# wangchou/whisper.coreml

Measured on AMD Instinct MI355X. Metric: xRT (audio-s/s) large-v3 beam=5 @1/2/4/8 GPU; p50 per-token decode ms, higher is better.
Workload: dtype fp16; 1 GPU; large-v3 beam=5 transcribe() of one 600 s file, 30 s clip grid, condition_on_previous_text=False, temperature=0; model=large-v3, global_batch=20, seq_len=448

## Files before the change

__graft_entry__.py:

```python
import os
import subprocess
import sys

REPO = os.path.dirname(os.path.abspath(__file__))
PKG = os.path.join(REPO, "whisper.coreml_amd")


def _paths():
    for p in (PKG, REPO):
        if p not in sys.path:
            sys.path.insert(0, p)


def build() -> None:
    env = dict(os.environ)
    env.setdefault("PYTORCH_ROCM_ARCH", "gfx950")
    jobs = str(min(8, os.cpu_count() or 4))
    subprocess.run(["make", "-C", PKG, "-j" + jobs, "ARCH=gfx950"], check=True, env=env)
    _paths()
    import whisper
    from whisper import backend_hip
    backend_hip.load_library()


def smoke() -> None:
    _paths()
    import numpy as np
    import torch

    import whisper
    from whisper import synthetic as S
    from whisper.decoding import DecodingOptions, decode
    from oracle import ref_whisper as R

    dims = S.MODEL_DIMS["micro"]
    sd = S.synthetic_state_dict(dims, 0)
    model = whisper.Whisper(whisper.ModelDimensions(**dims), "micro", device=0, dtype="fp32",
                            max_windows=1, max_group=1)
    model.load_state_dict(sd)
    audio = S.synthetic_audio(30.0, seed=3)

    mel = whisper.log_mel_spectrogram(audio, dims["n_mels"], padding=whisper.audio.N_SAMPLES)
    mel = whisper.pad_or_trim(mel[:, :3000], 3000)
    ref_mel = R.pad_or_trim(R.log_mel_spectrogram(audio, dims["n_mels"], padding=R.N_SAMPLES)[:, :3000]).numpy()
    err = float(np.abs(mel - ref_mel).max())
    assert err < 2e-3, f"log-mel max abs err {err}"

    om = R.OracleWhisper(dims, sd)
    xa_ref = om.encode(torch.from_numpy(mel)).numpy()
    model.ctx.mel_write(mel)
    model.ctx.encode([0], [3000])
    xa = model.ctx.audio_features(0)
    err = float(np.abs(xa - xa_ref.reshape(xa.shape)).max())
    assert err < 2e-3, f"audio features max abs err {err}"

    st = R.SpecialTokens.for_model(dims)
    om.set_audio(torch.from_numpy(xa_ref))
    ref_logits, _, _ = om.decoder_forward(torch.tensor([list(st.sot_sequence)]), 0, None)
    logits, _ = model.ctx.prefill_logits(0, list(st.sot_sequence))
    err = float(np.abs(logits[-1] - ref_logits[0, -1].numpy()).max())
    assert err < 2e-3, f"first-pass logits max abs err {err}"

    opts = DecodingOptions(language="en", sample_len=24, without_timestamps=True)
    res = decode(model, mel, opts)
    ref = R.decode(om, torch.from_numpy(mel), R.Options(sample_len=24, without_timestamps=True), st,
                   xa=torch.from_numpy(xa_ref))
    assert list(res.tokens) == list(ref.tokens), (res.tokens, ref.tokens)
    model.close()
    print(f"smoke ok: {len(res.tokens)} tokens match the oracle")


if __name__ == "__main__":
    build()
    if len(sys.argv) > 1 and sys.argv[1] == "smoke":
        smoke()
```

whisper.coreml_amd/csrc/wh_gemm.h:

```cpp
#pragma once
#include "wh_common.h"

namespace wh {

enum Epi {
  EPI_STORE = 0,
  EPI_STORE_GELU = 1,
  EPI_RESID = 2,
  EPI_GELU_POS = 3,
  EPI_HEADSPLIT = 4,
  EPI_QKV_DEC = 5,
  EPI_F32_COLS = 6,
  EPI_PARTIAL = 7,
  EPI_QKV_ENC = 8,
};

struct GemmArgs {
  const void* X = nullptr;
  const void* W = nullptr;
  const float* bias = nullptr;
  int M = 0, N = 0, K = 0;
  int ldx = 0;
  int x_group_rows = 1 << 30;
  int64_t x_group_stride = 0;
  void* out = nullptr;
  float* out_f32 = nullptr;
  int ldo = 0;
  int64_t out_group_stride = 0;
  int out_row_off = 0;
  const float* pos = nullptr;
  int hs_state = 0, hs_heads = 0, hs_T = 0, hs_nslots = 0, hs_slot0 = 0;
  const int* row_win = nullptr;
  const int* row_slot = nullptr;
  const int* row_pos = nullptr;
  void* kc = nullptr;
  void* vc = nullptr;
  int kv_beams = 0, kv_ctx = 0;
  const int* x_rows = nullptr;
  int ksplit = 1;
  int mt_block = 0;
  int row_groups = 1;
  const float* xf32 = nullptr;
  const float* ln_g = nullptr;
  const float* ln_b = nullptr;
  float ln_eps = 1e-5f;
  float* p1_slab = nullptr;
  int* p1_cnt = nullptr;
  int p1_slabs = 0;
  int p1_defer = 0;
  const float* res_slab = nullptr;
  const float* res_bias = nullptr;
  float* x_out = nullptr;
  int slab_half = 0;
};

template <typename T, int EPI>
WH_DEV void epilogue_store(const GemmArgs& a, int m, int gi, int ri, int n, float4_t v) {
  if constexpr (EPI == EPI_STORE || EPI == EPI_STORE_GELU) {
    if constexpr (EPI == EPI_STORE_GELU) {
#pragma unroll
      for (int j = 0; j < 4; ++j) v[j] = gelu_f(v[j]);
    }
    T* o = reinterpret_cast<T*>(a.out) + (int64_t)gi * a.out_group_stride + (int64_t)(ri + a.out_row_off) * a.ldo + n;
    store4(o, v[0], v[1], v[2], v[3]);
  } else if constexpr (EPI == EPI_RESID) {
    float* o = a.out_f32 + (int64_t)m * a.ldo + n;
    float4_t c = load4f(o);
    c += v;
    store4(o, c[0], c[1], c[2], c[3]);
  } else if constexpr (EPI == EPI_GELU_POS) {
    const float4_t p = load4f(a.pos + (int64_t)ri * a.N + n);
    float* o = a.out_f32 + (int64_t)m * a.ldo + n;
    store4(o, gelu_f(v[0]) + p[0], gelu_f(v[1]) + p[1], gelu_f(v[2]) + p[2], gelu_f(v[3]) + p[3]);
  } else if constexpr (EPI == EPI_HEADSPLIT) {
    const int l2 = n / a.hs_state, c = n - l2 * a.hs_state, h = c >> 6, d = c & 63;
    const int64_t blk = (((int64_t)l2 * a.hs_nslots + a.hs_slot0 + gi) * a.hs_heads + h) * a.hs_T * 64;
    T* o = reinterpret_cast<T*>(a.out) + blk;
    if ((l2 & 1) == 0) {
      store4(o + (int64_t)ri * 64 + d, v[0], v[1], v[2], v[3]);
    } else {
#pragma unroll
      for (int j = 0; j < 4; ++j) o[xv_index(d + j, ri)] = from_f32<T>(v[j]);
    }
  } else if constexpr (EPI == EPI_QKV_ENC) {
    if (n < 2 * a.hs_state) {
      T* o = reinterpret_cast<T*>(a.out) + (int64_t)gi * a.out_group_stride + (int64_t)ri * a.ldo + n;
      store4(o, v[0], v[1], v[2], v[3]);
    } else {
      const int c = n - 2 * a.hs_state, h = c >> 6, d = c & 63;
      const int q = ri & 31;
      const int pt = (ri & ~31) + 8 * ((q & 15) >> 2) + 4 * (q >> 4) + (q & 3);
      T* o = reinterpret_cast<T*>(a.vc) + (((int64_t)gi * a.hs_heads + h) * 64 + d) * a.hs_T + pt;
#pragma unroll
      for (int j = 0; j < 4; ++j) o[(int64_t)j * a.hs_T] = from_f32<T>(v[j]);
    }
  } else if constexpr (EPI == EPI_QKV_DEC) {
    const int ns = a.hs_state;
    if (n < ns) {
      store4(reinterpret_cast<T*>(a.out) + (int64_t)m * a.ldo + n, v[0], v[1], v[2], v[3]);
    } else {
      const int which = n >= 2 * ns;
      const int c = n - ns * (1 + which), h = c >> 6, d = c & 63;
      const int w = a.row_win[m], sl = a.row_slot[m], p = a.row_pos[m];
      const int64_t idx = ((((int64_t)w * a.kv_beams + sl) * a.hs_heads + h) * a.kv_ctx + p) * 64 + d;
      T* base = reinterpret_cast<T*>(which ? a.vc : a.kc);
      store4(base + idx, v[0], v[1], v[2], v[3]);
    }
  }
}

template <typename T, int EPI, int MI, int NI, int MG, typename RowF, typename ColF>
WH_DEV void tile_epilogue(const GemmArgs& a, const float4_t (&acc)[MI][NI], RowF mrow, ColF ncol) {
  static_assert(MI % MG == 0, "row-tile groups");
  constexpr bool LD = EPI == EPI_RESID || EPI == EPI_GELU_POS;
  float4_t bv[NI];
#pragma unroll
  for (int ni = 0; ni < NI; ++ni) bv[ni] = a.bias ? load4f(a.bias + ncol(ni)) : (float4_t){0.f, 0.f, 0.f, 0.f};
#pragma unroll
  for (int g0 = 0; g0 < MI; g0 += MG) {
    float4_t xv[LD ? MG : 1][LD ? NI : 1];
    if constexpr (LD) {
#pragma unroll
      for (int j = 0; j < MG; ++j) {
        const int m = mrow(g0 + j);
        const int gi = m / a.x_group_rows, ri = m - gi * a.x_group_rows;
#pragma unroll
        for (int ni = 0; ni < NI; ++ni) {
          xv[j][ni] = (float4_t){0.f, 0.f, 0.f, 0.f};
          if (m < a.M) {
            if constexpr (EPI == EPI_RESID) xv[j][ni] = load4f(a.out_f32 + (int64_t)m * a.ldo + ncol(ni));
            else xv[j][ni] = load4f(a.pos + (int64_t)ri * a.N + ncol(ni));
          }
        }
      }
    }
#pragma unroll
    for (int j = 0; j < MG; ++j) {
      const int m = mrow(g0 + j);
      if (m >= a.M) continue;
      const int gi = m / a.x_group_rows, ri = m - gi * a.x_group_rows;
#pragma unroll
      for (int ni = 0; ni < NI; ++ni) {
        const int n = ncol(ni);
        float4_t v = acc[g0 + j][ni];
        if (a.bias) v += bv[ni];
        if constexpr (EPI == EPI_RESID) {
          float4_t c = xv[j][ni];
          c += v;
          store4(a.out_f32 + (int64_t)m * a.ldo + n, c[0], c[1], c[2], c[3]);
        } else if constexpr (EPI == EPI_GELU_POS) {
          const float4_t p = xv[j][ni];
          store4(a.out_f32 + (int64_t)m * a.ldo + n, gelu_f(v[0]) + p[0], gelu_f(v[1]) + p[1], gelu_f(v[2]) + p[2],
                 gelu_f(v[3]) + p[3]);
        } else {
          epilogue_store<T, EPI>(a, m, gi, ri, n, v);
        }
      }
    }
  }
}

template <typename T>
int launch_gemm(const GemmArgs& a, int epi, hipStream_t st);
template <typename T>
int launch_gemm_tiles(const GemmArgs& a, int epi, int tile_sel, hipStream_t st);

template <typename T>
int launch_proj_partial(const GemmArgs& a, int max_z, hipStream_t st, int* z_out, hipEvent_t ev0 = nullptr,
                        hipEvent_t ev1 = nullptr);

bool proj1_supported(int R, int n);
template <typename T>
int launch_proj1(const GemmArgs& a, int epi, bool ln, hipStream_t st, hipEvent_t ev0 = nullptr,
                 hipEvent_t ev1 = nullptr);

int gemv_ksplit(int M, int N, int K, int max_z = 16, int mt_block = 0);

}
```

whisper.coreml_amd/csrc/wh_gemm.hip:

```cpp
#include "wh_gemm.h"

#include <algorithm>
#include <type_traits>
#include <cstdlib>

namespace wh {

constexpr int TBM = 128, TBN = 128, TKB = 128;
constexpr int TROW = TKB + 16;

template <typename T, int EPI, int TBN_ = TBN, int KZ = 1>
__global__ __launch_bounds__(256, 2) void k_gemm_tile(GemmArgs a) {
  static_assert(KZ == 1 || KZ == 2, "two K halves at most (their sum commutes)");
  constexpr int BK = TKB / (int)sizeof(T);
  constexpr int KS = BK / 32;
  constexpr int WCH = TBN_ / 32;
  constexpr int NI = TBN_ / 32;
  __shared__ __attribute__((aligned(16))) char smem[2][(TBM + TBN_) * TROW];

  const int ntn = a.N / TBN_;
  const int ntm = (a.M + TBM - 1) / TBM;
  const int rid = xcd_remap(blockIdx.x, ntm * ntn * KZ);
  const int bid = rid / KZ, kz = rid - bid * KZ;
  const int tm = bid / ntn, tn = bid % ntn;
// ... 59 lines not shown
      for (int mi = 0; mi < 4; ++mi)
#pragma unroll
        for (int ni = 0; ni < NI; ++ni) mfma_step(acc[mi][ni], wf[ni], xf[mi]);
    }
  };

  const int nk = a.K / BK / KZ;
  gload(0, ra);
  gload(min(1, nk - 1), rb);
  sstore(0, ra);
  lds_barrier();
  for (int kt = 0; kt < nk; kt += 2) {
    gload(min(kt + 2, nk - 1), ra);
    compute(0);
    if (kt + 1 < nk) sstore(1, rb);
    lds_barrier();
    if (kt + 1 >= nk) break;
    gload(min(kt + 3, nk - 1), rb);
    compute(1);
    if (kt + 2 < nk) sstore(0, ra);
    lds_barrier();
  }

  if constexpr (KZ > 1) {
    constexpr int NE = 4 * NI;
    const int slot = bid * 4 + wave, nslot = ntm * ntn * 4;
    const auto rs = wt_rsrc(a.p1_slab);
    auto off = [&](int z, int e) { return (((z * nslot + slot) * NE + e) * 64 + lane) * 16; };
#pragma unroll
    for (int mi = 0; mi < 4; ++mi)
#pragma unroll
      for (int ni = 0; ni < NI; ++ni) wt_store4(rs, off(kz, mi * NI + ni), acc[mi][ni]);
    asm volatile("s_waitcnt vmcnt(0)" ::: "memory");
    int ticket = 0;
    if (lane == 0) ticket = __hip_atomic_fetch_add(a.p1_cnt + slot, 1, __ATOMIC_RELAXED, __HIP_MEMORY_SCOPE_AGENT);
    ticket = __shfl(ticket, 0, 64);
    if (ticket != KZ - 1) return;
    __builtin_amdgcn_fence(__ATOMIC_ACQUIRE, "wavefront");
    if (lane == 0) __hip_atomic_store(a.p1_cnt + slot, 0, __ATOMIC_RELAXED, __HIP_MEMORY_SCOPE_AGENT);
    float4_t pv[4][NI];
#pragma unroll
    for (int mi = 0; mi < 4; ++mi)
#pragma unroll
      for (int ni = 0; ni < NI; ++ni)
        pv[mi][ni] = __builtin_bit_cast(float4_t, __builtin_amdgcn_raw_buffer_load_b128(rs, off(1 - kz, mi * NI + ni), 0, 16));
#pragma unroll
    for (int mi = 0; mi < 4; ++mi)
#pragma unroll
      for (int ni = 0; ni < NI; ++ni) acc[mi][ni] += pv[mi][ni];
  }

  tile_epilogue<T, EPI, 4, NI, 2>(
      a, acc, [&](int mi) { return m0 + wr * 64 + mi * 16 + r; },
      [&](int ni) { return n0 + wc * (TBN_ / 2) + ni * 16 + 4 * g; });
}

namespace g256 {
constexpr int BM = 256, BN = 256, BK = 64;
constexpr int STAGE = 16384;
constexpr int BUF = 4 * STAGE;
enum { SA0 = 0, SA1 = 1, SB0 = 2, SB1 = 3 };
}

WH_DEV void raw_barrier() {
  asm volatile("" ::: "memory");
  __builtin_amdgcn_sched_barrier(0);
  __builtin_amdgcn_s_barrier();
  __builtin_amdgcn_sched_barrier(0);
  asm volatile("" ::: "memory");
}

WH_DEV void glds16(const char* src, char* lds) {
  __builtin_amdgcn_global_load_lds((__attribute__((address_space(1))) void*)(src),
                                   (__attribute__((address_space(3))) void*)(lds), 16, 0, 0);
}

template <int EPI, int MF = 16>
__global__ __launch_bounds__(512, 1) void k_gemm_256(GemmArgs a) {
  using namespace g256;
  __shared__ __attribute__((aligned(1024))) char smem[2 * BUF];

  const int ntn = a.N / BN;
  const int ntm = (a.M + BM - 1) / BM;
  const int bid = xcd_remap(blockIdx.x, ntm * ntn);
  const int tm = bid / ntn, tn = bid % ntn;
  const int m0 = tm * BM, n0 = tn * BN;
  const int tid = threadIdx.x, lane = tid & 63, wave = tid >> 6;
  const int wr = wave >> 2, wc = wave & 3;
  const int r = lane & 15, g = lane >> 4;

  const int srow = lane >> 2;
  const int schunk = (lane & 3) ^ ((lane >> 5) << 1);
  const half_t* X = reinterpret_cast<const half_t*>(a.X);
  const half_t* W = reinterpret_cast<const half_t*>(a.W);
  const char* src[4];
#pragma unroll
  for (int h = 0; h < 2; ++h) {
    int m = m0 + (wave >> 2) * 128 + h * 64 + (wave & 3) * 16 + srow;
    if (m >= a.M) m = a.M - 1;
    const int gi = m / a.x_group_rows, ri = m - gi * a.x_group_rows;
    src[SA0 + h] = reinterpret_cast<const char*>(X + (int64_t)gi * a.x_group_stride + (int64_t)ri * a.ldx) + schunk * 16;
    const int n = n0 + (wave >> 1) * 64 + h * 32 + (wave & 1) * 16 + srow;
    src[SB0 + h] = reinterpret_cast<const char*>(W + (int64_t)n * a.K) + schunk * 16;
  }
  auto stage = [&](int buf, int st, int kt) {
    const char* s = src[st] + kt * (BK * 2);
    char* d = smem + buf * BUF + st * STAGE + wave * 2048;
    glds16(s, d);
    glds16(s + 64, d + 1024);
  };

  const int roff = r * 64 + ((g ^ ((r >> 3) << 1)) << 4);
  Frag<half_t> af[4][2], bf[2][2];
  auto read_a = [&](int buf, int h) {
    const char* base = smem + buf * BUF + (SA0 + h) * STAGE + wr * 8192 + roff;
#pragma unroll
    for (int mi = 0; mi < 4; ++mi)
#pragma unroll
      for (int ks = 0; ks < 2; ++ks) af[mi][ks].v = *reinterpret_cast<const half8_t*>(base + (mi * 2 + ks) * 1024);
  };
  auto read_b = [&](int buf, int h) {
    const char* base = smem + buf * BUF + (SB0 + h) * STAGE + wc * 4096 + roff;
#pragma unroll
    for (int j = 0; j < 2; ++j)
#pragma unroll
      for (int ks = 0; ks < 2; ++ks) bf[j][ks].v = *reinterpret_cast<const half8_t*>(base + (j * 2 + ks) * 1024);
  };

  const int rr = lane & 15, hb = (lane >> 4) & 1, kh = lane >> 5;
  const int coff0 = rr * 64 + (((0 + kh) ^ ((rr >> 3) << 1)) << 4);
  const int coff1 = rr * 64 + (((2 + kh) ^ ((rr >> 3) << 1)) << 4);
  Frag<half_t> af32[MF == 32 ? 2 : 1][4], bf32[4];
  auto read_a32 = [&](int buf, int h) {
    const char* base = smem + buf * BUF + (SA0 + h) * STAGE + wr * 8192;
#pragma unroll
    for (int t = 0; t < 2; ++t)
#pragma unroll
      for (int st = 0; st < 4; ++st)
        af32[t][st].v = *reinterpret_cast<const half8_t*>(base + ((t * 2 + hb) * 2 + (st >> 1)) * 1024 +
                                                             ((st & 1) ? coff1 : coff0));
  };
  auto read_b32 = [&](int buf, int h) {
    const char* base = smem + buf * BUF + (SB0 + h) * STAGE + wc * 4096;
#pragma unroll
    for (int st = 0; st < 4; ++st)
      bf32[st].v = *reinterpret_cast<const half8_t*>(base + (hb * 2 + (st >> 1)) * 1024 + ((st & 1) ? coff1 : coff0));
  };
  typedef float f32x16_t __attribute__((ext_vector_type(16)));
  f32x16_t acc32[MF == 32 ? 4 : 1][2];
  float4_t acc[MF == 32 ? 1 : 8][4];
  if constexpr (MF == 32) {
#pragma unroll
    for (int i = 0; i < 4; ++i)
#pragma unroll
      for (int j = 0; j < 2; ++j) acc32[i][j] = (f32x16_t){};
  } else {
#pragma unroll
    for (int i = 0; i < 8; ++i)
#pragma unroll
      for (int j = 0; j < 4; ++j) acc[i][j] = (float4_t){0.f, 0.f, 0.f, 0.f};
  }
  auto rd_a = [&](int buf, int h) {
    if constexpr (MF == 32) read_a32(buf, h);
    else read_a(buf, h);
  };
  auto rd_b = [&](int buf, int h) {
    if constexpr (MF == 32) read_b32(buf, h);
    else read_b(buf, h);
  };

  auto mfma_quadrant = [&](int mh, int nh) {
    asm volatile("s_waitcnt lgkmcnt(0)" ::: "memory");
    __builtin_amdgcn_s_setprio(1);
    if constexpr (MF == 32) {
#pragma unroll
      for (int t = 0; t < 2; ++t)
#pragma unroll
        for (int st = 0; st < 4; ++st)
          acc32[mh * 2 + t][nh] =
              __builtin_amdgcn_mfma_f32_32x32x16_f16(bf32[st].v, af32[t][st].v, acc32[mh * 2 + t][nh], 0, 0, 0);
    } else {
#pragma unroll
      for (int mi = 0; mi < 4; ++mi)
#pragma unroll
        for (int j = 0; j < 2; ++j)
#pragma unroll
          for (int ks = 0; ks < 2; ++ks) mfma_step(acc[mh * 4 + mi][nh * 2 + j], bf[j][ks], af[mi][ks]);
    }
    __builtin_amdgcn_s_setprio(0);
  };

  const int nk = a.K / BK;
  auto ktile = [&](auto bufc, int t) {
    constexpr int buf = decltype(bufc)::value;
    const bool s1 = t + 1 < nk, s2 = t + 2 < nk;
    rd_b(buf, 0);
    rd_a(buf, 0);
    if (s1) stage(buf ^ 1, SA1, t + 1);
    raw_barrier();
    mfma_quadrant(0, 0);
    raw_barrier();
    rd_b(buf, 1);
    if (s1) stage(buf ^ 1, SB0, t + 1);
    raw_barrier();
    mfma_quadrant(0, 1);
    raw_barrier();
    rd_a(buf, 1);
    if (s2) stage(buf, SA0, t + 2);
    raw_barrier();
    mfma_quadrant(1, 1);
    raw_barrier();
    rd_b(buf, 0);
    if (s2) {
      stage(buf, SB1, t + 2);
      asm volatile("s_waitcnt vmcnt(4)" ::: "memory");
    } else {
      asm volatile("s_waitcnt vmcnt(0)" ::: "memory");
    }
    raw_barrier();
    mfma_quadrant(1, 0);
    raw_barrier();
  };

  stage(0, SA0, 0);
  stage(0, SB1, 0);
  stage(0, SA1, 0);
  stage(0, SB0, 0);
  stage(1, SA0, 1);
  stage(1, SB1, 1);
  asm volatile("s_waitcnt vmcnt(4)" ::: "memory");
  raw_barrier();
  if (wr == 1) raw_barrier();
  for (int t = 0; t < nk; t += 2) {
    ktile(std::integral_constant<int, 0>(), t);
    ktile(std::integral_constant<int, 1>(), t + 1);
  }
  if (wr == 0) raw_barrier();

  if constexpr (MF == 32) {
    float4_t a4[4][8];
#pragma unroll
    for (int mt = 0; mt < 4; ++mt)
#pragma unroll
      for (int j = 0; j < 8; ++j) {
        const int nt = j >> 2, q = j & 3;
        a4[mt][j] = (float4_t){acc32[mt][nt][4 * q], acc32[mt][nt][4 * q + 1], acc32[mt][nt][4 * q + 2],
                               acc32[mt][nt][4 * q + 3]};
      }
    tile_epilogue<half_t, EPI, 4, 8, 2>(
        a, a4, [&](int mt) { return m0 + wr * 128 + mt * 32 + (lane & 31); },
        [&](int j) { return n0 + wc * 64 + (j >> 2) * 32 + 8 * (j & 3) + 4 * kh; });
  } else {
    tile_epilogue<half_t, EPI, 8, 4, 4>(
        a, acc, [&](int mi) { return m0 + wr * 128 + mi * 16 + r; },
        [&](int ni) { return n0 + wc * 64 + ni * 16 + 4 * g; });
  }
}

template <typename T, int MT, int EPI>
__global__ __launch_bounds__(512) void k_gemv_rows(GemmArgs a) {
  constexpr int NW = 8;
  constexpr int U = sizeof(T) == 2 ? 4 : 2;
  __shared__ float red[NW][MT][64][4];
  const int tid = threadIdx.x, lane = tid & 63, wave = tid >> 6;
  const int r = lane & 15, g = lane >> 4;
  const int n0 = blockIdx.x * 16;
  const int mb = blockIdx.y * (16 * MT);
  const T* X = reinterpret_cast<const T*>(a.X);
  const T* W = reinterpret_cast<const T*>(a.W);

  const int kz = blockIdx.z;
  const int S = a.K / 32;
  const int kb = (S * kz / (int)gridDim.z) * 32;
  const int Kc = (S * (kz + 1) / (int)gridDim.z) * 32 - kb;
  int nrow = n0 + r;
  if (nrow >= a.N) nrow = a.N - 1;
  const T* wp = W + (int64_t)nrow * a.K + kb + 8 * g;
  const T* xp[MT];
#pragma unroll
  for (int mt = 0; mt < MT; ++mt) {
    int m = mb + mt * 16 + r;
    if (m >= a.M) m = a.M - 1;
    const int xr = a.x_rows ? a.x_rows[m] : m;
    xp[mt] = X + (int64_t)xr * a.ldx + kb + 8 * g;
  }
  float4_t acc[MT];
#pragma unroll
  for (int mt = 0; mt < MT; ++mt) acc[mt] = (float4_t){0.f, 0.f, 0.f, 0.f};

  const int nsteps = Kc / 32;
  const int last = nsteps - 1;
  for (int b0 = wave; b0 < nsteps; b0 += NW * U) {
    Frag<T> wf[U];
    Frag<T> xf[U][MT];
#pragma unroll
    for (int u = 0; u < U; ++u) {
      const int su = min(b0 + NW * u, last) * 32;
      frag_load(wf[u], wp + su);
#pragma unroll
      for (int mt = 0; mt < MT; ++mt) frag_load(xf[u][mt], xp[mt] + su);
    }
#pragma unroll
    for (int u = 0; u < U; ++u) {
      if (b0 + NW * u < nsteps) {
#pragma unroll
        for (int mt = 0; mt < MT; ++mt) mfma_step(acc[mt], wf[u], xf[u][mt]);
      }
    }
  }
#pragma unroll
  for (int mt = 0; mt < MT; ++mt)
    *reinterpret_cast<float4_t*>(&red[wave][mt][lane][0]) = acc[mt];
  __syncthreads();
  for (int idx = tid; idx < MT * 64; idx += 512) {
    const int mt = idx >> 6, ln = idx & 63;
    float4_t v = *reinterpret_cast<float4_t*>(&red[0][mt][ln][0]);
#pragma unroll
    for (int w = 1; w < NW; ++w) v += *reinterpret_cast<float4_t*>(&red[w][mt][ln][0]);
    const int m = mb + mt * 16 + (ln & 15);
    const int n = n0 + 4 * (ln >> 4);
    if (m >= a.M || n >= a.N) continue;
    if (EPI == EPI_F32_COLS) {
      float* o = a.out_f32 + (int64_t)m * a.ldo;
#pragma unroll
      for (int j = 0; j < 4; ++j)
        if (n + j < a.N) o[n + j] = v[j] + (a.bias ? a.bias[n + j] : 0.f);
      continue;
    }
    if (EPI == EPI_PARTIAL) {
      store4(a.out_f32 + ((int64_t)kz * a.M + m) * a.ldo + n, v[0], v[1], v[2], v[3]);
      continue;
    }
    if (a.bias) v += load4f(a.bias + n);
    epilogue_store<T, EPI>(a, m, 0, m, n, v);
  }
}


// ... 422 lines not shown
        for (int mt = 0; mt < MT; ++mt) {
          Frag<T> xf;
          frag_load(xf, reinterpret_cast<const T*>(xs + (mt * 16 + r) * XS_ROW) + s * 32 + 8 * g);
          mfma_step(acc[mt], wf[s], xf);
        }
      }
    }
    __syncthreads();
    if (more) {
#pragma unroll
      for (int s = 0; s < KS; ++s) wf[s] = wn[s];
    }
  }
  const int n = n0 + 4 * g;
#pragma unroll
  for (int mt = 0; mt < MT; ++mt) {
    const int m = mb + mt * 16 + r;
    if (m >= a.M || n >= a.N) continue;
    float4_t v = acc[mt];
    if (EPI == EPI_F32_COLS) {
#if WH_WT
      const auto rs = wt_rsrc(a.out_f32);
#pragma unroll
      for (int j = 0; j < 4; ++j)
        if (n + j < a.N) wt_store1(rs, (m * a.ldo + n + j) * 4, v[j] + (a.bias ? a.bias[n + j] : 0.f));
#else
      float* o = a.out_f32 + (int64_t)m * a.ldo;
#pragma unroll
      for (int j = 0; j < 4; ++j)
        if (n + j < a.N) o[n + j] = v[j] + (a.bias ? a.bias[n + j] : 0.f);
#endif
      continue;
    }
    if (EPI == EPI_PARTIAL) {
#if WH_WT
      wt_store4(wt_rsrc(a.out_f32), (int)((((int64_t)kz * a.M + m) * a.ldo + n) * 4), v);
#else
      store4(a.out_f32 + ((int64_t)kz * a.M + m) * a.ldo + n, v[0], v[1], v[2], v[3]);
#endif
      continue;
    }
    if (a.bias) v += load4f(a.bias + n);
    epilogue_store<T, EPI>(a, m, 0, m, n, v);
  }
}

static int rows_per_block(int M, int mt_block) {
  const int mt = (M + 15) / 16;
  if (mt_block > 0) return std::min(mt_block, std::min(mt, 8));
  return mt >= 8 ? 8 : mt;
}

int gemv_ksplit(int M, int N, int K, int max_z, int mt_block) {
  const char* env = tune_env("WHISPER_HIP_GEMV_WGS");
  const int target = env ? atoi(env) : 256;
  const int mt = (M + 15) / 16;
  const bool xpath = mt >= 3;
  const int rp = rows_per_block(M, mt_block);
  const int wgs = (xpath ? (N + 63) / 64 : (N + 15) / 16) * ((M + 16 * rp - 1) / (16 * rp));
  const int steps = K / 32;
  int best = 1;
  for (int z = 1; z <= 16 && z <= max_z && z <= steps; ++z)
    if (wgs * z <= target) best = z;
  return best;
}

template <typename T>
int launch_gemm_tiles(const GemmArgs& a, int epi, int tile_sel, hipStream_t st);

template <typename T>
int launch_gemm(const GemmArgs& a, int epi, hipStream_t st) {
  return launch_gemm_tiles<T>(a, epi, 256, st);
}

template <typename T>
int launch_gemm_tiles(const GemmArgs& a, int epi, int tile_sel, hipStream_t st) {
  if (a.M <= 0) return 0;
  const bool big = a.M > 128 && (a.N % TBN) == 0 && (a.K % (TKB / (int)sizeof(T))) == 0 && epi != EPI_F32_COLS &&
                   epi != EPI_PARTIAL && a.x_rows == nullptr;
  const bool t256 = big && sizeof(T) == 2 && (tile_sel == 256 || tile_sel == 257) && a.M >= 256 && (a.N % g256::BN) == 0 &&
                    (a.K % (2 * g256::BK)) == 0 && epi != EPI_QKV_DEC &&
                    ((a.M + g256::BM - 1) / g256::BM) * (a.N / g256::BN) >= 256;
  if (t256) {
    const int nwg = ((a.M + g256::BM - 1) / g256::BM) * (a.N / g256::BN);
    switch (epi) {
#define CASE(E)                                                   \
  case E:                                                         \
    if (tile_sel == 257) k_gemm_256<E, 32><<<nwg, 512, 0, st>>>(a), wh_launched("k_gemm_256"); \
    else k_gemm_256<E><<<nwg, 512, 0, st>>>(a), wh_launched("k_gemm_256");                    \
    break;
      CASE(EPI_STORE) CASE(EPI_STORE_GELU) CASE(EPI_RESID) CASE(EPI_GELU_POS) CASE(EPI_HEADSPLIT) CASE(EPI_QKV_ENC)
#undef CASE
      default: return -1;
    }
  } else if (big) {
    const int ntm = (a.M + TBM - 1) / TBM;
    const bool half = ntm * (a.N / TBN) < 256 && (a.N % 64) == 0 && tile_sel != 129;
    const int nwg = ntm * (a.N / (half ? 64 : TBN));
    const bool kz2 = half && sizeof(T) == 2 && (epi == EPI_RESID || epi == EPI_GELU_POS) && a.p1_slab && a.p1_cnt &&
                     (a.K / (TKB / (int)sizeof(T))) % 2 == 0 && (int64_t)nwg * 64 <= a.p1_slabs && tile_sel != 128;
    if (kz2) {
      if (epi == EPI_RESID) k_gemm_tile<T, EPI_RESID, 64, 2><<<2 * nwg, 256, 0, st>>>(a), wh_launched("k_gemm_tile");
      else k_gemm_tile<T, EPI_GELU_POS, 64, 2><<<2 * nwg, 256, 0, st>>>(a), wh_launched("k_gemm_tile");
      return 0;
    }
    switch (epi) {
#define CASE(E)                                                       \
  case E:                                                             \
    if (half) k_gemm_tile<T, E, 64><<<nwg, 256, 0, st>>>(a), wh_launched("k_gemm_tile");          \
    else k_gemm_tile<T, E><<<nwg, 256, 0, st>>>(a), wh_launched("k_gemm_tile");                   \
    break;
      CASE(EPI_STORE) CASE(EPI_STORE_GELU) CASE(EPI_RESID) CASE(EPI_GELU_POS) CASE(EPI_HEADSPLIT) CASE(EPI_QKV_DEC)
      CASE(EPI_QKV_ENC)
#undef CASE
      default: return -1;
    }
  } else {
    if (a.K % 32) return -2;
    if (a.x_group_rows != a.M && a.x_group_rows != 0 && a.x_group_rows < a.M) return -3;
    const int mt = (a.M + 15) / 16;
    const int rows_per = rows_per_block(a.M, a.mt_block);
    const int ks = epi == EPI_PARTIAL ? a.ksplit : 1;
    if (ks < 1 || ks > a.K / 32) return -4;
    static const bool vocab_small = [] {
      const char* e = tune_env("WHISPER_HIP_VOCAB_SMALL");
      return !(e && e[0] == '0');
    }();
    if (a.xf32 && !(vocab_small && epi == EPI_F32_COLS && a.N >= 16384 && a.M <= 8 && a.K <= 1280 && a.K % 32 == 0 &&
                    !a.x_rows))
      return -6;
    static const bool vocab1 = [] {
      const char* e = tune_env("WHISPER_HIP_VOCAB1");
      return !(e && e[0] == '0');
    }();
    if (sizeof(T) == 2 && vocab1 && a.xf32 && a.K == 1280 && !a.bias && a.M <= 8 && (a.N + 15) / 16 <= 256 * 13) {
      constexpr int D = 6;
      const int lds = 8 * (1280 * 2 + 16) + 13 * 8 * 64 * 16;
      static bool attr = hipFuncSetAttribute(reinterpret_cast<const void*>(&k_vocab1<D>),
                                             hipFuncAttributeMaxDynamicSharedMemorySize, 160 * 1024) == hipSuccess;
      if (!attr) return -5;
      k_vocab1<D><<<256, 512, lds, st>>>(a), wh_launched("k_vocab1");
      return 0;
    }
    const int vxrow = a.K * (int)sizeof(T) + 16;
    const int vrg_max = std::min(64, (152 * 1024) / vxrow);
    const int vgrp = (a.M + vrg_max - 1) / vrg_max;
    if (vocab_small && epi == EPI_F32_COLS && !a.bias && a.N >= 16384 && a.M <= (sizeof(T) == 2 ? 32 : 16) && vgrp <= 4 &&
        a.K <= 1280 && a.K % 32 == 0) {
      const int rg = (a.M + vgrp - 1) / vgrp, mtv = (rg + 15) / 16;
      const int lds = rg * vxrow;
      const int grid = vgrp * std::max(1, std::min(256 / vgrp, (a.N + 127) / 128));
      GemmArgs av = a;
      av.row_groups = vgrp;
      auto go = [&](auto mtc) {
        constexpr int MTV = decltype(mtc)::value;
        static bool attr = hipFuncSetAttribute(reinterpret_cast<const void*>(&k_vocab_small<T, MTV>),
                                               hipFuncAttributeMaxDynamicSharedMemorySize, 160 * 1024) == hipSuccess;
        if (!attr) return -5;
        k_vocab_small<T, MTV><<<grid, 512, lds, st>>>(av), wh_launched("k_vocab_small");
        return 0;
      };
      switch (mtv) {
        case 1: return go(std::integral_constant<int, 1>());
        case 2: return go(std::integral_constant<int, 2>());
        case 3: return go(std::integral_constant<int, 3>());
        default: return go(std::integral_constant<int, 4>());
      }
    }
    if (sizeof(T) == 2 && vocab_small && epi == EPI_F32_COLS && !a.bias && a.N >= 16384 && a.M > 32 && a.M <= 112 &&
        !a.xf32 &&
        a.K == 1280 && a.M * (a.K + 16) <= 150 * 1024) {
      const int nt = (a.N + 15) / 16;
      const int grid = std::max((nt + 15) / 16, std::min(256, nt));
// ... 83 lines not shown
```

whisper.coreml_amd/csrc/wh_runtime.hip:

```cpp
#include <hip/hip_runtime.h>

#include <algorithm>
#include <chrono>
#include <cmath>
#include <cstdio>
#include <cstring>
#include <set>
#include <string>
#include <vector>

#include "whisper_hip.h"
#include "wh_align.h"
#include "wh_audio.h"
#include "wh_gemm.h"
#include "wh_host.h"
#include "wh_kernels.h"

using namespace wh;

static thread_local std::string g_release_error;

namespace {

constexpr int CTX = 448;
constexpr int HCTX = CTX + 1;
constexpr int NSPLIT = 8;
static int enc_chunk() {
  static const int v = [] {
    const char* e = tune_env("WHISPER_HIP_ENC_CHUNK");
    const int c = e ? atoi(e) : 16;
    return c >= 1 && c <= 64 ? c : 16;
  }();
  return v;
}
constexpr int PRE_ROWS = 1024;
constexpr int MROWS = 3008;
constexpr int H1ROWS = 3002;
constexpr int KC = 9;
constexpr int EKZ_TILES(int n) { return 12 * (n / 64); }
constexpr int RSPLIT = 16;

struct Arena {
  char* base = nullptr;
  size_t cap = 0, off = 0;
  void* take(size_t bytes) {
    off = (off + 255) & ~size_t(255);
    void* p = base + off;
    off += bytes;
    return off <= cap ? p : nullptr;
  }
};

template <typename T>
struct EncLayer {
  float *ln1_g, *ln1_b, *bqkv, *bo, *ln2_g, *ln2_b, *b1, *b2;
  T *wqkv, *wo, *w1, *w2;
};
template <typename T>
struct DecLayer {
  float *ln1_g, *ln1_b, *bqkv, *bo, *lnx_g, *lnx_b, *bqx, *box, *ln2_g, *ln2_b, *b1, *b2;
  T *wqkv, *wo, *wqx, *wox, *w1, *w2;
  T* wqx_f = nullptr;
};

}

struct wh_ctx {
  virtual std::string step_kernels(int n_win, int group) const = 0;
  virtual ~wh_ctx() {}
  virtual int load(const std::string& name, const float* data, const int64_t* shape, int ndim) = 0;
  virtual int finalize() = 0;
  virtual int encode(int n_win, const int64_t* seeks, const int* segs) = 0;
  virtual int read_xa(int slot, float* out) = 0;
  virtual int read_ckv(int slot, int layer, float* k, float* v) = 0;
  virtual int decode_begin(int n_win, const wh_decode_opts* o, const int* init, const int* n_init, int max_init,
                           const int* sot_index, const int* slots) = 0;
  virtual int decode_steps(int max_steps, int* n_done) = 0;
  virtual int step_prefill(int n_win, int G, const int* init, const int* n_init, int max_init, const int* sot_index,
                           float* lg) = 0;
  virtual int step_tokens(const int* tok, const int* offsets, float* lg) = 0;
  virtual int reorder_kv(const int* src) = 0;
  virtual int decode_read(int slot, int* tokens, float* slp, int* len, int* fin_n, int* fin_tok, int* fin_len,
                          float* fin_score, float* nsp) = 0;
  virtual int prefill_logits(int slot, const int* tokens, int n, float* logits, const int* ah, int na, float* aqk) = 0;
  virtual int align(int slot, const int* tokens, int n, int n_sot, int num_frames, const int* ah, int na, int medfilt,
                    float* probs, int* path, int* plen) = 0;
  virtual int align_batch(int n_win, const int* slots, const int* tokens, const int* n_tokens, int n_sot,
                          const int* num_frames, const int* ah, int na, int medfilt, float* probs, int* paths,
                          int* plens) = 0;
  virtual int dtw(const float* x, int N, int M, int* path, int* plen) = 0;
  virtual int time_stage(int what, int iters, double* ms) = 0;
  virtual int share_weights_from(wh_ctx* src) = 0;
  int sharers = 0;
  wh_ctx* shares_from = nullptr;
  std::vector<float> token_ms;
  double stats[WH_N_STATS] = {0};
  AudioFront audio;
  int n_mels = 0;
  int n_vocab = 0;
  std::vector<wh::BiasRec> bias_tab;
  int maxc = 5;
  int maxc_stride = 1;
  int device = 0;
};

namespace {

template <typename T>
struct Ctx : public wh_ctx {
  wh_dims d;
  int ns, nh, La, Ld, V, K1p;
  int Wcap, Gcap;
  hipStream_t st = nullptr;
  Arena wa;
// ... 1710 lines not shown
```

Baseline: 759.9 audio-s/s.

## Make 256-tile encoder GEMM persistent with cross-tile prefetch and larger encode chunk

Converts the k_gemm_256 kernel into a persistent kernel. The grid is capped at the CU count, and each workgroup loops over several output tiles. While the last k-tiles of the current tile are still in flight, it stages the first k-tiles of the next tile, so global loads overlap the epilogue and the prologue. The default encoder chunk rises from 16 to 20 windows, the tile_sel 257 path is restricted to EPI_STORE, and asm barriers are added to keep lane-derived offsets and bias from being kept live in registers. The trade-offs are more register pressure, possible load imbalance when the tile count is not a multiple of the CU count, and more workspace for the larger chunk.

```diff
diff --git a/__graft_entry__.py b/__graft_entry__.py
--- a/__graft_entry__.py
+++ b/__graft_entry__.py
@@ -17,6 +17,7 @@
     env.setdefault("PYTORCH_ROCM_ARCH", "gfx950")
     jobs = str(min(8, os.cpu_count() or 4))
     subprocess.run(["make", "-C", PKG, "-j" + jobs, "ARCH=gfx950"], check=True, env=env)
+    subprocess.run(["make", "-C", PKG, "ARCH=gfx950", "tools/gemm_bench"], check=True, env=env)
     _paths()
     import whisper
     from whisper import backend_hip
diff --git a/profiles/enc_pingpong/enc_trace.py b/profiles/enc_pingpong/enc_trace.py
--- /dev/null
+++ b/profiles/enc_pingpong/enc_trace.py
@@ -0,0 +1,25 @@
+import os
+import sys
+
+REPO = os.path.dirname(os.path.dirname(os.path.dirname(os.path.abspath(__file__))))
+
+
+def main():
+    sys.path.insert(0, os.path.join(REPO, "whisper.coreml_amd"))
+    import whisper
+    from whisper import synthetic as S
+    dims = S.MODEL_DIMS["large-v3"]
+    model = whisper.Whisper(whisper.ModelDimensions(**dims), "large-v3", device=0, dtype="fp16",
+                            max_windows=20, max_group=5)
+    model.load_state_dict(S.synthetic_state_dict(dims, 0))
+    audio = S.synthetic_audio(600.0, seed=1000)
+    model.ctx.log_mel(audio, padding=480000, n_mels=dims["n_mels"], normalize=True)
+    for _ in range(2):
+        model.ctx.encode([3000 * i for i in range(20)], [3000] * 20)
+    model.ctx.sync()
+    model.close()
+    print("ok")
+
+
+if __name__ == "__main__":
+    main()
diff --git a/whisper.coreml_amd/csrc/wh_gemm.h b/whisper.coreml_amd/csrc/wh_gemm.h
--- a/whisper.coreml_amd/csrc/wh_gemm.h
+++ b/whisper.coreml_amd/csrc/wh_gemm.h
@@ -40,6 +40,7 @@
   int ksplit = 1;
   int mt_block = 0;
   int row_groups = 1;
+  int tile_grid = 0;
   const float* xf32 = nullptr;
   const float* ln_g = nullptr;
   const float* ln_b = nullptr;
@@ -117,6 +118,8 @@
 #pragma unroll
   for (int ni = 0; ni < NI; ++ni) bv[ni] = a.bias ? load4f(a.bias + ncol(ni)) : (float4_t){0.f, 0.f, 0.f, 0.f};
 #pragma unroll
+  for (int ni = 0; ni < NI; ++ni) asm volatile("" : "+v"(bv[ni]));
+#pragma unroll
   for (int g0 = 0; g0 < MI; g0 += MG) {
     float4_t xv[LD ? MG : 1][LD ? NI : 1];
     if constexpr (LD) {
diff --git a/whisper.coreml_amd/csrc/wh_gemm.hip b/whisper.coreml_amd/csrc/wh_gemm.hip
--- a/whisper.coreml_amd/csrc/wh_gemm.hip
+++ b/whisper.coreml_amd/csrc/wh_gemm.hip
@@ -165,27 +165,25 @@
 
   const int ntn = a.N / BN;
   const int ntm = (a.M + BM - 1) / BM;
-  const int bid = xcd_remap(blockIdx.x, ntm * ntn);
-  const int tm = bid / ntn, tn = bid % ntn;
-  const int m0 = tm * BM, n0 = tn * BN;
+  const int ntiles = ntm * ntn, nwg = gridDim.x;
   const int tid = threadIdx.x, lane = tid & 63, wave = tid >> 6;
   const int wr = wave >> 2, wc = wave & 3;
   const int r = lane & 15, g = lane >> 4;
+  const int nk = a.K / BK;
 
   const int srow = lane >> 2;
   const int schunk = (lane & 3) ^ ((lane >> 5) << 1);
   const half_t* X = reinterpret_cast<const half_t*>(a.X);
   const half_t* W = reinterpret_cast<const half_t*>(a.W);
   const char* src[4];
-#pragma unroll
-  for (int h = 0; h < 2; ++h) {
+  auto tile_src = [&](int m0, int n0, int h, const char*& sa, const char*& sb) {
     int m = m0 + (wave >> 2) * 128 + h * 64 + (wave & 3) * 16 + srow;
     if (m >= a.M) m = a.M - 1;
     const int gi = m / a.x_group_rows, ri = m - gi * a.x_group_rows;
-    src[SA0 + h] = reinterpret_cast<const char*>(X + (int64_t)gi * a.x_group_stride + (int64_t)ri * a.ldx) + schunk * 16;
+    sa = reinterpret_cast<const char*>(X + (int64_t)gi * a.x_group_stride + (int64_t)ri * a.ldx) + schunk * 16;
     const int n = n0 + (wave >> 1) * 64 + h * 32 + (wave & 1) * 16 + srow;
-    src[SB0 + h] = reinterpret_cast<const char*>(W + (int64_t)n * a.K) + schunk * 16;
-  }
+    sb = reinterpret_cast<const char*>(W + (int64_t)n * a.K) + schunk * 16;
+  };
   auto stage = [&](int buf, int st, int kt) {
     const char* s = src[st] + kt * (BK * 2);
     char* d = smem + buf * BUF + st * STAGE + wave * 2048;
@@ -193,7 +191,7 @@
     glds16(s + 64, d + 1024);
   };
 
-  const int roff = r * 64 + ((g ^ ((r >> 3) << 1)) << 4);
+  int roff, coff0, coff1;
   Frag<half_t> af[4][2], bf[2][2];
   auto read_a = [&](int buf, int h) {
     const char* base = smem + buf * BUF + (SA0 + h) * STAGE + wr * 8192 + roff;
@@ -210,9 +208,15 @@
       for (int ks = 0; ks < 2; ++ks) bf[j][ks].v = *reinterpret_cast<const half8_t*>(base + (j * 2 + ks) * 1024);
   };
 
-  const int rr = lane & 15, hb = (lane >> 4) & 1, kh = lane >> 5;
-  const int coff0 = rr * 64 + (((0 + kh) ^ ((rr >> 3) << 1)) << 4);
-  const int coff1 = rr * 64 + (((2 + kh) ^ ((rr >> 3) << 1)) << 4);
+  const int hb = (lane >> 4) & 1;
+  auto set_read_offsets = [&] {
+    int tl = lane;
+    asm volatile("" : "+v"(tl));
+    const int tr = tl & 15, tg = tl >> 4, tkh = tl >> 5;
+    roff = tr * 64 + ((tg ^ ((tr >> 3) << 1)) << 4);
+    coff0 = tr * 64 + (((0 + tkh) ^ ((tr >> 3) << 1)) << 4);
+    coff1 = tr * 64 + (((2 + tkh) ^ ((tr >> 3) << 1)) << 4);
+  };
   Frag<half_t> af32[MF == 32 ? 2 : 1][4], bf32[4];
   auto read_a32 = [&](int buf, int h) {
     const char* base = smem + buf * BUF + (SA0 + h) * STAGE + wr * 8192;
@@ -232,17 +236,6 @@
   typedef float f32x16_t __attribute__((ext_vector_type(16)));
   f32x16_t acc32[MF == 32 ? 4 : 1][2];
   float4_t acc[MF == 32 ? 1 : 8][4];
-  if constexpr (MF == 32) {
-#pragma unroll
-    for (int i = 0; i < 4; ++i)
-#pragma unroll
-      for (int j = 0; j < 2; ++j) acc32[i][j] = (f32x16_t){};
-  } else {
-#pragma unroll
-    for (int i = 0; i < 8; ++i)
-#pragma unroll
-      for (int j = 0; j < 4; ++j) acc[i][j] = (float4_t){0.f, 0.f, 0.f, 0.f};
-  }
   auto rd_a = [&](int buf, int h) {
     if constexpr (MF == 32) read_a32(buf, h);
     else read_a(buf, h);
@@ -273,29 +266,27 @@
     __builtin_amdgcn_s_setprio(0);
   };
 
-  const int nk = a.K / BK;
-  auto ktile = [&](auto bufc, int t) {
+  auto ktile = [&](auto bufc, int k1, int k2, bool s1, bool s2) {
     constexpr int buf = decltype(bufc)::value;
-    const bool s1 = t + 1 < nk, s2 = t + 2 < nk;
     rd_b(buf, 0);
     rd_a(buf, 0);
-    if (s1) stage(buf ^ 1, SA1, t + 1);
+    if (s1) stage(buf ^ 1, SA1, k1);
     raw_barrier();
     mfma_quadrant(0, 0);
     raw_barrier();
     rd_b(buf, 1);
-    if (s1) stage(buf ^ 1, SB0, t + 1);
+    if (s1) stage(buf ^ 1, SB0, k1);
     raw_barrier();
     mfma_quadrant(0, 1);
     raw_barrier();
     rd_a(buf, 1);
-    if (s2) stage(buf, SA0, t + 2);
+    if (s2) stage(buf, SA0, k2);
     raw_barrier();
     mfma_quadrant(1, 1);
     raw_barrier();
     rd_b(buf, 0);
     if (s2) {
-      stage(buf, SB1, t + 2);
+      stage(buf, SB1, k2);
       asm volatile("s_waitcnt vmcnt(4)" ::: "memory");
     } else {
       asm volatile("s_waitcnt vmcnt(0)" ::: "memory");
@@ -305,6 +296,12 @@
     raw_barrier();
   };
 
+  int v = blockIdx.x;
+  {
+    const int bid = xcd_remap(v, ntiles);
+#pragma unroll
+    for (int h = 0; h < 2; ++h) tile_src((bid / ntn) * BM, (bid % ntn) * BN, h, src[SA0 + h], src[SB0 + h]);
+  }
   stage(0, SA0, 0);
   stage(0, SB1, 0);
   stage(0, SA1, 0);
@@ -313,30 +310,66 @@
   stage(1, SB1, 1);
   asm volatile("s_waitcnt vmcnt(4)" ::: "memory");
   raw_barrier();
-  if (wr == 1) raw_barrier();
-  for (int t = 0; t < nk; t += 2) {
-    ktile(std::integral_constant<int, 0>(), t);
-    ktile(std::integral_constant<int, 1>(), t + 1);
-  }
-  if (wr == 0) raw_barrier();
-
-  if constexpr (MF == 32) {
-    float4_t a4[4][8];
-#pragma unroll
-    for (int mt = 0; mt < 4; ++mt)
-#pragma unroll
-      for (int j = 0; j < 8; ++j) {
-        const int nt = j >> 2, q = j & 3;
-        a4[mt][j] = (float4_t){acc32[mt][nt][4 * q], acc32[mt][nt][4 * q + 1], acc32[mt][nt][4 * q + 2],
-                               acc32[mt][nt][4 * q + 3]};
-      }
-    tile_epilogue<half_t, EPI, 4, 8, 2>(
-        a, a4, [&](int mt) { return m0 + wr * 128 + mt * 32 + (lane & 31); },
-        [&](int j) { return n0 + wc * 64 + (j >> 2) * 32 + 8 * (j & 3) + 4 * kh; });
-  } else {
-    tile_epilogue<half_t, EPI, 8, 4, 4>(
-        a, acc, [&](int mi) { return m0 + wr * 128 + mi * 16 + r; },
-        [&](int ni) { return n0 + wc * 64 + ni * 16 + 4 * g; });
+  for (; v < ntiles; v += nwg) {
+    const int bid = xcd_remap(v, ntiles);
+    const int m0 = (bid / ntn) * BM, n0 = (bid % ntn) * BN;
+    const bool more = v + nwg < ntiles;
+    set_read_offsets();
+    if constexpr (MF == 32) {
+#pragma unroll
+      for (int i = 0; i < 4; ++i)
+#pragma unroll
+        for (int j = 0; j < 2; ++j) acc32[i][j] = (f32x16_t){};
+    } else {
+#pragma unroll
+      for (int i = 0; i < 8; ++i)
+#pragma unroll
+        for (int j = 0; j < 4; ++j) acc[i][j] = (float4_t){0.f, 0.f, 0.f, 0.f};
+    }
+    if (wr == 1) raw_barrier();
+    for (int t = 0; t < nk - 2; t += 2) {
+      ktile(std::integral_constant<int, 0>(), t + 1, t + 2, true, true);
+      ktile(std::integral_constant<int, 1>(), t + 2, t + 3, true, true);
+    }
+    const char* nsrc[4];
+    if (more) {
+      const int nb = xcd_remap(v + nwg, ntiles);
+#pragma unroll
+      for (int h = 0; h < 2; ++h)
+        tile_src((nb / ntn) * BM, (nb % ntn) * BN, h, nsrc[SA0 + h], nsrc[SB0 + h]);
+      src[SA0] = nsrc[SA0];
+      src[SB1] = nsrc[SB1];
+    }
+    ktile(std::integral_constant<int, 0>(), nk - 1, 0, true, more);
+    if (more) {
+      src[SA1] = nsrc[SA1];
+      src[SB0] = nsrc[SB0];
+    }
+    ktile(std::integral_constant<int, 1>(), 0, 1, more, more);
+    if (wr == 0) raw_barrier();
+
+    int el = lane;
+    asm volatile("" : "+v"(el));
+    const int er = el & 15, eg = el >> 4, ekh = el >> 5;
+    if constexpr (MF == 32) {
+      float4_t a4[4][8];
+#pragma unroll
+      for (int mt = 0; mt < 4; ++mt)
+#pragma unroll
+        for (int j = 0; j < 8; ++j) {
+          const int nt = j >> 2, q = j & 3;
+          a4[mt][j] = (float4_t){acc32[mt][nt][4 * q], acc32[mt][nt][4 * q + 1], acc32[mt][nt][4 * q + 2],
+                                 acc32[mt][nt][4 * q + 3]};
+        }
+      tile_epilogue<half_t, EPI, 4, 8, 2>(
+          a, a4, [&](int mt) { return m0 + wr * 128 + mt * 32 + (el & 31); },
+          [&](int j) { return n0 + wc * 64 + (j >> 2) * 32 + 8 * (j & 3) + 4 * ekh; });
+    } else {
+      constexpr int MG = (EPI == EPI_RESID || EPI == EPI_GELU_POS) ? 2 : 4;
+      tile_epilogue<half_t, EPI, 8, 4, MG>(
+          a, acc, [&](int mi) { return m0 + wr * 128 + mi * 16 + er; },
+          [&](int ni) { return n0 + wc * 64 + ni * 16 + 4 * eg; });
+    }
   }
 }
 
@@ -925,13 +958,23 @@
                     (a.K % (2 * g256::BK)) == 0 && epi != EPI_QKV_DEC &&
                     ((a.M + g256::BM - 1) / g256::BM) * (a.N / g256::BN) >= 256;
   if (t256) {
-    const int nwg = ((a.M + g256::BM - 1) / g256::BM) * (a.N / g256::BN);
+    const int ntiles = ((a.M + g256::BM - 1) / g256::BM) * (a.N / g256::BN);
+    static const int cus = [] {
+      int dev = 0, n = 0;
+      if (hipGetDevice(&dev) != hipSuccess ||
+          hipDeviceGetAttribute(&n, hipDeviceAttributeMultiprocessorCount, dev) != hipSuccess || n < 1)
+        n = 256;
+      return n;
+    }();
+    const int nwg = std::min(ntiles, a.tile_grid > 0 ? a.tile_grid : cus);
+    if (tile_sel == 257) {
+      if (epi != EPI_STORE) return -1;
+      k_gemm_256<EPI_STORE, 32><<<nwg, 512, 0, st>>>(a), wh_launched("k_gemm_256");
+      return 0;
+    }
     switch (epi) {
-#define CASE(E)                                                   \
-  case E:                                                         \
-    if (tile_sel == 257) k_gemm_256<E, 32><<<nwg, 512, 0, st>>>(a), wh_launched("k_gemm_256"); \
-    else k_gemm_256<E><<<nwg, 512, 0, st>>>(a), wh_launched("k_gemm_256");                    \
-    break;
+#define CASE(E) \
+  case E: k_gemm_256<E><<<nwg, 512, 0, st>>>(a), wh_launched("k_gemm_256"); break;
       CASE(EPI_STORE) CASE(EPI_STORE_GELU) CASE(EPI_RESID) CASE(EPI_GELU_POS) CASE(EPI_HEADSPLIT) CASE(EPI_QKV_ENC)
 #undef CASE
       default: return -1;
diff --git a/whisper.coreml_amd/csrc/wh_runtime.hip b/whisper.coreml_amd/csrc/wh_runtime.hip
--- a/whisper.coreml_amd/csrc/wh_runtime.hip
+++ b/whisper.coreml_amd/csrc/wh_runtime.hip
@@ -28,8 +28,8 @@
 static int enc_chunk() {
   static const int v = [] {
     const char* e = tune_env("WHISPER_HIP_ENC_CHUNK");
-    const int c = e ? atoi(e) : 16;
-    return c >= 1 && c <= 64 ? c : 16;
+    const int c = e ? atoi(e) : 20;
+    return c >= 1 && c <= 64 ? c : 20;
   }();
   return v;
 }
```

New measurement: 760.4 audio-s/s (median of 4 runs). Within noise of the previous version (+0.1%).
